# NagsTheProgrammer/WindGNN

Measured on NVIDIA B200. Metric: gcn_gru_forward_sequences_per_s, higher is better.
Workload: dtype f32

## Files before the change

windgnn_b200/csrc/abi.cu:

```cuda

#include "../../include/windgnn_b200.h"

#include <cmath>
#include <cstdarg>
#include <cstdio>
#include <cstdlib>
#include <cstring>
#include <mutex>
#include <vector>

#include "gcn.cuh"
#include "gcn_bwd.cuh"
#include "gcn_bwd_rows.cuh"
#include "gcn_rows.cuh"
#include "gcn_sparse.cuh"
#include "gcn_sparse_plan.cuh"
#include "gemm_kb.cuh"
#include "gru_bwd.cuh"
#include "inproj.cuh"
#include "inproj_tc2.cuh"
#include "recur.cuh"
#include "recur_tc.cuh"
#include "recur_unit.cuh"
#include "sgemm.cuh"
// ... 35 lines not shown

constexpr size_t kAlign = 256;
size_t align_up(size_t v) { return (v + kAlign - 1) / kAlign * kAlign; }

enum GcnKind { kGcnRows, kGcn13x7, kGcn13x4, kGcn16x4, kGcnSparsePlan, kGcnSparseLanes };
enum RecurKind { kRecurTc, kRecurUnit, kRecurWide };

struct Plan {
    int T, S, Fi, Fh, Fo, H;
    long long chunk;
    int I, G;
    int IP;
    int NPB;
    int GP;
    int KP;
    int NPR;
    int n_bias;
    bool sparse;
    GcnKind gcn;
    size_t gcn_smem;
    int gcn_rb;
    int gcn_threads;
    size_t off_sqw, off_sqsteps, off_sqpairs;
    bool tc;
    wg::Tc2Shape tc2;
    RecurKind recur;
    bool regw;
    bool whu;
    int ru_wpg, ru_ht;
    int ru_rmax;
    int rc_ts;
    size_t rc_smem;
    size_t off_wp, off_bias, off_wht, off_whu, off_bhn, off_u, off_gi, off_z, total;
    size_t off_whh_hi, off_whh_lo;
};

long long default_chunk(long long B, size_t bytes_per_seq) {
    long long c = (long long)wg::kNumSMs * wg::kRcBT;
    const size_t cap = (size_t)6 << 30;
    if ((size_t)c * bytes_per_seq > cap) {
        c = (long long)(cap / bytes_per_seq) / wg::kRcBT * wg::kRcBT;
        if (c < wg::kRcBT) c = wg::kRcBT;
    }
    return B < c ? (B < 1 ? 1 : B) : c;
}

// ... 92 lines not shown
    const int wrows = p.tc && p.tc2.NP > p.NPB ? p.tc2.NP : p.NPB;
    p.n_bias = wrows > 512 ? wrows : 512;
    p.off_wp = o;   o = align_up(o + (p.tc ? wg::tc2_w_halves(p.tc2) * 2 : (size_t)p.NPB * p.IP * 4));
    p.off_bias = o; o = align_up(o + (size_t)p.n_bias * 4);
    p.off_wht = o;  o = align_up(o + (size_t)p.KP * p.NPR * 4);
    p.off_whu = o;
    if (p.whu) o = align_up(o + (size_t)p.KP * 3 * wg::recur_u_hp2(H) * 4);
    p.off_bhn = o;  o = align_up(o + (size_t)p.KP * 4);
    const bool tc_recur = p.recur == kRecurTc;
    p.off_whh_hi = o; if (tc_recur) o = align_up(o + wg::recur_tc_w_halves(H) * 2);
    p.off_whh_lo = o; if (tc_recur) o = align_up(o + wg::recur_tc_w_halves(H) * 2);
    const size_t rows = table_rows > 0 ? (size_t)forecast_piece_rows(p, table_rows) : (size_t)p.chunk * T;
    const size_t rows_tiled = (rows + wg::kUTileRows - 1) / wg::kUTileRows * wg::kUTileRows;
    p.off_u = o;    o = align_up(o + rows_tiled * p.IP * 4);
    const size_t rows_gi =
        table_rows > 0 ? (size_t)table_rows : (size_t)((p.chunk + wg::kRtSeqs - 1) / wg::kRtSeqs * wg::kRtSeqs) * T;
    p.off_gi = o;   o = align_up(o + rows_gi * p.GP * 4);
    p.off_z = o;    if (sparse) o = align_up(o + (rows + wg::kNumSMs) * (size_t)S * Fo * 4);
    const bool sq = p.gcn == kGcnSparsePlan;
    p.off_sqw = o;     if (sq) o = align_up(o + sizeof(wg::SqWeights));
    p.off_sqsteps = o;
    p.off_sqpairs = o + (size_t)wg::round_up(wg::ceil_div(S, 32), 4) * sizeof(int);
    if (sq) o = align_up(o + wg::sq_plan_bytes(S));
    p.total = o;
    return WG_OK;
}

int plan_launch(Plan& p) {
    const long long rows = p.chunk * p.T;
    switch (p.gcn) {
    case kGcnRows:
        p.gcn_smem = wg::gcn_rows_smem_floats(p.S) * 4;
        p.gcn_threads = wg::gcn_rows_warps(p.S) * 32;
        break;
    case kGcnSparsePlan: {
        p.gcn_smem = wg::gcn_sparse_plan_smem_bytes(p.S, p.Fi, p.Fo);
        const long long rt = (rows + wg::kSpThreads - 1) / wg::kSpThreads * wg::kSpThreads;
        if (rt / 32 > 65535) return fail(WG_ERR_UNSUPPORTED, "sparse GCN: chunk of %lld rows too large", rows);
        break;
    }
    case kGcnSparseLanes:
        if (p.Fi > wg::kSpF || p.Fo > wg::kSpF)
            return fail(WG_ERR_UNSUPPORTED, "sparse GCN: F_in / F_out must be <= %d (got %d / %d)", wg::kSpF, p.Fi, p.Fo);
        p.gcn_smem = ((size_t)2 * p.Fh * wg::kSpF + p.Fh) * 4;
        if (p.gcn_smem > (size_t)wg::kMaxSmemOptin)
            return fail(WG_ERR_UNSUPPORTED, "sparse GCN: hidden width %d too large", p.Fh);
// ... 88 lines not shown
    WG_CUDA(cudaOccupancyMaxActiveBlocksPerMultiprocessor(&per_sm, kern, wg::kGcnThreads, smem));
    if (per_sm < 1) per_sm = 1;
    const long long nblocks = (R + RB - 1) / RB;
    long long grid = (long long)wg::kNumSMs * per_sm;
    if (grid > nblocks) grid = nblocks;
    if (grid < 1) return WG_OK;
    kern<<<(unsigned)grid, wg::kGcnThreads, smem, st>>>(X, adj, W1, b1, W2, b2, out, R, S, Fi, Fh, Fo, ldo, RB);
    WG_CUDA(cudaGetLastError());
    return WG_OK;
}

template <int LAYERS, bool TILED>
int launch_gcn_dense(GcnKind k, int RB, size_t smem, const float* X, const float* adj, const float* W1,
                     const float* b1, const float* W2, const float* b2, float* out, long long R, int S, int Fi, int Fh,
                     int Fo, int ldo, cudaStream_t st) {
#define WG_GCN(FP, SG, EX) \
    launch_gcn_t<FP, SG, EX, LAYERS, TILED>(X, adj, W1, b1, W2, b2, out, R, S, Fi, Fh, Fo, ldo, RB, smem, st)
    if (k == kGcn13x7) return WG_GCN(13, 7, true);
    if (k == kGcn13x4) return WG_GCN(13, 4, true);
    return WG_GCN(16, 4, false);
#undef WG_GCN
}

int launch_gcn_rows(const Plan& p, const float* X, const float* adj, const float* W1, const float* b1,
                    const float* W2, const float* b2, float* out, long long R, cudaStream_t st) {
    WG_CUDA(cudaFuncSetAttribute(wg::gcn_rows_kernel, cudaFuncAttributeMaxDynamicSharedMemorySize, (int)p.gcn_smem));
    int per_sm = 0;
    WG_CUDA(cudaOccupancyMaxActiveBlocksPerMultiprocessor(&per_sm, wg::gcn_rows_kernel, p.gcn_threads, p.gcn_smem));
    if (per_sm < 1) per_sm = 1;
    const long long nblocks = (R + wg::kGrRows - 1) / wg::kGrRows;
    long long grid = (long long)wg::kNumSMs * per_sm;
    if (grid > nblocks) grid = nblocks;
    if (grid < 1) return WG_OK;
    wg::gcn_rows_kernel<<<(unsigned)grid, p.gcn_threads, p.gcn_smem, st>>>(X, adj, W1, b1, W2, b2, out, R, p.S, p.IP);
    WG_CUDA(cudaGetLastError());
    return WG_OK;
}

struct Graph {
    const float* adj;
    const int* rowptr;
    const int* colidx;
    const float* vals;
};

int launch_gcn_sparse(const Plan& p, void* ws, const Graph& g, const float* x, const float* w1, const float* b1,
                      const float* w2, const float* b2, long long rows, cudaStream_t st) {
    if (rows < 1) return WG_OK;
    if (p.gcn == kGcnSparsePlan) {
        const bool narrow = p.Fi <= 13 && p.Fo <= 13, exact = p.Fi == 13 && p.Fo == 13;
        auto kern = exact ? wg::gcn_sparse_plan_kernel<13, true>
                          : narrow ? wg::gcn_sparse_plan_kernel<13, false> : wg::gcn_sparse_plan_kernel<16, false>;
        WG_CUDA(cudaFuncSetAttribute(kern, cudaFuncAttributeMaxDynamicSharedMemorySize, (int)p.gcn_smem));
        const unsigned grid = (unsigned)(rows < wg::kNumSMs ? rows : wg::kNumSMs);
        float* urow = ws_ptr<float>(ws, p.off_z);
        float* zscr = urow + (size_t)rows * p.S * p.Fo;
        kern<<<grid, wg::kSqThreads, p.gcn_smem, st>>>(x, g.rowptr, g.colidx, g.vals, ws_ptr<int>(ws, p.off_sqsteps),
// ... 10 lines not shown
    }
    const long long tiles = (rows + wg::kSpThreads - 1) / wg::kSpThreads;
    int chunks = (int)((4LL * wg::kNumSMs * 4 + tiles - 1) / tiles);
    if (chunks < 1) chunks = 1;
    if (chunks > p.S) chunks = p.S;
    const int s_chunk = (p.S + chunks - 1) / chunks;
    const dim3 grid((unsigned)tiles, (unsigned)((p.S + s_chunk - 1) / s_chunk));
    WG_CUDA(cudaFuncSetAttribute(wg::gcn_sparse_l1_kernel, cudaFuncAttributeMaxDynamicSharedMemorySize,
                                 (int)p.gcn_smem));
    wg::gcn_sparse_l1_kernel<<<grid, wg::kSpThreads, p.gcn_smem, st>>>(x, g.rowptr, g.colidx, g.vals, w1, b1, w2,
                                                                       ws_ptr<float>(ws, p.off_z), rows, p.S, p.Fi,
                                                                       p.Fh, p.Fo, s_chunk);
    WG_CUDA(cudaGetLastError());
    wg::gcn_sparse_l2_kernel<<<grid, wg::kSpThreads, 0, st>>>(ws_ptr<float>(ws, p.off_z), g.rowptr, g.colidx, g.vals,
                                                             b2, ws_ptr<float>(ws, p.off_u), rows, p.S, p.Fo, p.IP,
                                                             s_chunk);
    WG_CUDA(cudaGetLastError());
    return WG_OK;
}

int launch_gcn(const Plan& p, void* ws, const Graph& g, const float* x, const float* w1, const float* b1,
               const float* w2, const float* b2, long long rows, cudaStream_t st) {
    float* u = ws_ptr<float>(ws, p.off_u);
    if (p.gcn == kGcnRows) return launch_gcn_rows(p, x, g.adj, w1, b1, w2, b2, u, rows, st);
    if (p.sparse) return launch_gcn_sparse(p, ws, g, x, w1, b1, w2, b2, rows, st);
    return launch_gcn_dense<2, true>(p.gcn, p.gcn_rb, p.gcn_smem, x, g.adj, w1, b1, w2, b2, u, rows, p.S, p.Fi, p.Fh,
                                     p.Fo, p.IP, st);
}

int launch_inproj_tc(const Plan& p, void* ws, long long rows, cudaStream_t st, float* gi) {
    const long long m_tiles = (rows + wg::kT2BM - 1) / wg::kT2BM;
    if (m_tiles < 1) return WG_OK;
    const wg::Tc2Shape& t = p.tc2;
    WG_CUDA(cudaFuncSetAttribute(wg::inproj_tc2_kernel, cudaFuncAttributeMaxDynamicSharedMemorySize,
                                 (int)t.smem_bytes));
    const long long tiles = m_tiles * t.n_nt;
    const unsigned grid = (unsigned)(tiles < wg::kNumSMs ? tiles : wg::kNumSMs);
    wg::inproj_tc2_kernel<<<grid, wg::kT2Threads, t.smem_bytes, st>>>(
        ws_ptr<float>(ws, p.off_u), ws_ptr<__half>(ws, p.off_wp), ws_ptr<float>(ws, p.off_bias), gi, rows, p.IP,
        t.KP, p.GP, t.n_nt, t.N_each, t.stages);
    WG_CUDA(cudaGetLastError());
    return WG_OK;
}

int launch_inproj(const Plan& p, void* ws, long long rows, cudaStream_t st, float* gi) {
    if (p.tc) return launch_inproj_tc(p, ws, rows, st, gi);
    const long long m_tiles = (rows + wg::kIpBM - 1) / wg::kIpBM;
// ... 135 lines not shown
                                                           ws_ptr<__half>(ws, p.off_whh_lo), p.H);
        WG_CUDA(cudaGetLastError());
    }
    return WG_OK;
}

int run_chunk(const Plan& p, void* ws, const Graph& g, const float* x, const float* w1, const float* b1,
              const float* w2, const float* b2, float* out, long long Bc, cudaStream_t st, float* gsave = nullptr,
              int ldsave = 0) {
    const long long rows = Bc * p.T;
    int rc = launch_gcn(p, ws, g, x, w1, b1, w2, b2, rows, st);
    if (rc) return rc;
    rc = launch_inproj(p, ws, rows, st, ws_ptr<float>(ws, p.off_gi));
    if (rc) return rc;
    return launch_recur(p, ws, out, Bc, st, gsave, ldsave);
}

constexpr int kMaxDevices = 64;

std::mutex g_sq_mu;
struct SqDeviceState { cudaEvent_t ev = nullptr; cudaStream_t last = nullptr; bool recorded = false; };
SqDeviceState g_sq_dev[kMaxDevices];

int prepare_sparse(const Plan& p, void* ws, const Graph& g, const float* w1, const float* b1, const float* w2,
                   const float* b2, int device, cudaStream_t st) {
    if (device >= kMaxDevices) return fail(WG_ERR_BAD_ARG, "device index %d out of range", device);
    wg::SqWeights* stage = ws_ptr<wg::SqWeights>(ws, p.off_sqw);
    wg::sq_pack_weights_kernel<<<32, 256, 0, st>>>(w1, b1, w2, b2, stage, p.Fi, p.Fh, p.Fo);
    WG_CUDA(cudaGetLastError());
    const int wbs = wg::ceil_div(p.S, 32);
    wg::csr_plan_kernel<<<wg::ceil_div(wbs, 4), 128, 0, st>>>(g.rowptr, g.colidx, g.vals, p.S,
                                                             ws_ptr<int>(ws, p.off_sqsteps),
                                                             ws_ptr<int2>(ws, p.off_sqpairs));
    WG_CUDA(cudaGetLastError());
    SqDeviceState& d = g_sq_dev[device];
    cudaStreamCaptureStatus cap = cudaStreamCaptureStatusNone;
    cudaStreamIsCapturing(st, &cap);
    if (cap == cudaStreamCaptureStatusNone && d.recorded && d.last != st) WG_CUDA(cudaStreamWaitEvent(st, d.ev, 0));
    WG_CUDA(cudaMemcpyToSymbolAsync(wg::c_sq, stage, sizeof(wg::SqWeights), 0, cudaMemcpyDeviceToDevice, st));
    return WG_OK;
}
int finish_sparse(int device, cudaStream_t st) {
    SqDeviceState& d = g_sq_dev[device];
    cudaStreamCaptureStatus cap = cudaStreamCaptureStatusNone;
    cudaStreamIsCapturing(st, &cap);
    if (cap != cudaStreamCaptureStatusNone) return WG_OK;
    if (!d.ev) WG_CUDA(cudaEventCreateWithFlags(&d.ev, cudaEventDisableTiming));
    WG_CUDA(cudaEventRecord(d.ev, st));
    d.last = st;
    d.recorded = true;
    return WG_OK;
}

bool any_null(std::initializer_list<const void*> ps) {
    for (const void* q : ps)
        if (!q) return true;
    return false;
}

template <typename Stages>
int run_packed(const Plan& p, size_t need, const Graph& g, const float* x, const float* w1, const float* b1,
               const float* w2, const float* b2, const float* w_ih, const float* w_hh, const float* b_ih,
               const float* b_hh, const float* out, void* ws, size_t ws_bytes, int device, void* stream,
               Stages stages) {
    const bool no_graph = p.sparse ? any_null({g.rowptr, g.colidx, g.vals}) : !g.adj;
    if (no_graph || any_null({x, w1, b1, w2, b2, w_ih, w_hh, b_ih, b_hh, out}))
        return fail(WG_ERR_BAD_ARG, "null pointer argument");
    int rc = check_ws(ws, ws_bytes, need);
    if (rc) return rc;
    DeviceGuard dg(device);
    WG_CUDA(dg.err);
    cudaStream_t st = static_cast<cudaStream_t>(stream);
    if ((rc = launch_pack(p, ws, w_ih, w_hh, b_ih, b_hh, st))) return rc;
    const bool sq = p.gcn == kGcnSparsePlan;
    std::unique_lock<std::mutex> sq_lock(g_sq_mu, std::defer_lock);
    if (sq) {
        sq_lock.lock();
        if ((rc = prepare_sparse(p, ws, g, w1, b1, w2, b2, device, st))) return rc;
    }
    if ((rc = stages(st))) return rc;
    return sq ? finish_sparse(device, st) : WG_OK;
}

int forward(const Plan& p, size_t need, const Graph& g, const float* x, const float* w1, const float* b1,
            const float* w2, const float* b2, const float* w_ih, const float* w_hh, const float* b_ih,
            const float* b_hh, float* out, long long B, void* ws, size_t ws_bytes, int device, void* stream,
            float* gsave = nullptr, int ldsave = 0) {
    if (B == 0) return WG_OK;
    auto stages = [&](cudaStream_t st) {
        const size_t x_seq = (size_t)p.T * p.S * p.Fi, o_seq = (size_t)p.T * p.H;
        for (long long b0 = 0; b0 < B; b0 += p.chunk) {
            const long long Bc = (B - b0) < p.chunk ? (B - b0) : p.chunk;
            const int rc = run_chunk(p, ws, g, x + (size_t)b0 * x_seq, w1, b1, w2, b2, out + (size_t)b0 * o_seq, Bc,
                                     st, gsave ? gsave + (size_t)b0 * p.T * ldsave : nullptr, ldsave);
            if (rc) return rc;
        }
        return (int)WG_OK;
    };
    return run_packed(p, need, g, x, w1, b1, w2, b2, w_ih, w_hh, b_ih, b_hh, out, ws, ws_bytes, device, stream,
                      stages);
}

struct ForecastPlan {
    Plan p;
// ... 265 lines not shown
int wg_internal_fail(int code, const char* msg) { return fail(code, "%s", msg); }
const char* wg_last_error(void) { return g_err; }

size_t wg_gcn_gru_workspace_bytes(int64_t B, int T, int S, int F_in, int F_hid, int F_out, int H,
                                  int64_t chunk, int flags) {
    Plan p;
    if (make_plan(p, B, T, S, F_in, F_hid, F_out, H, chunk, false, flags)) return 0;
    return p.total;
}

int wg_stage_pack_f32(const float* w_ih, const float* w_hh, const float* b_ih, const float* b_hh, int T,
                      int S, int F_in, int F_hid, int F_out, int H, int64_t chunk, int flags, void* workspace,
                      size_t workspace_bytes, int device, void* stream) {
    if (any_null({w_ih, w_hh, b_ih, b_hh})) return fail(WG_ERR_BAD_ARG, "null parameter pointer");
    auto launch = [&](const Plan& p, cudaStream_t st) { return launch_pack(p, workspace, w_ih, w_hh, b_ih, b_hh, st); };
    return run_stage(0, T, S, F_in, F_hid, F_out, H, chunk, flags, workspace, workspace_bytes, device, stream, launch);
}

int wg_stage_gcn_f32(const float* adj, const float* x, const float* w1, const float* b1, const float* w2,
                     const float* b2, int64_t Bc, int T, int S, int F_in, int F_hid, int F_out, int H,
                     int64_t chunk, int flags, void* workspace, size_t workspace_bytes, int device, void* stream) {
    if (any_null({adj, x, w1, b1, w2, b2})) return fail(WG_ERR_BAD_ARG, "null pointer");
    auto launch = [&](const Plan& p, cudaStream_t st) {
        return launch_gcn(p, workspace, Graph{adj}, x, w1, b1, w2, b2, Bc * T, st);
    };
    return run_stage(Bc, T, S, F_in, F_hid, F_out, H, chunk, flags, workspace, workspace_bytes, device, stream, launch);
}

int wg_stage_inproj_f32(int64_t Bc, int T, int S, int F_in, int F_hid, int F_out, int H, int64_t chunk,
                        int flags, void* workspace, size_t workspace_bytes, int device, void* stream) {
    auto launch = [&](const Plan& p, cudaStream_t st) {
        return launch_inproj(p, workspace, Bc * T, st, ws_ptr<float>(workspace, p.off_gi));
    };
    return run_stage(Bc, T, S, F_in, F_hid, F_out, H, chunk, flags, workspace, workspace_bytes, device, stream, launch);
}

int wg_stage_recur_f32(float* out, int64_t Bc, int T, int S, int F_in, int F_hid, int F_out, int H,
                       int64_t chunk, int flags, void* workspace, size_t workspace_bytes, int device, void* stream) {
    if (!out) return fail(WG_ERR_BAD_ARG, "null output pointer");
    auto launch = [&](const Plan& p, cudaStream_t st) { return launch_recur(p, workspace, out, Bc, st, nullptr, 0); };
    return run_stage(Bc, T, S, F_in, F_hid, F_out, H, chunk, flags, workspace, workspace_bytes, device, stream, launch);
}

int wg_gcn_gru_forward_f32(const float* adj, const float* x, const float* w1, const float* b1,
                           const float* w2, const float* b2, const float* w_ih, const float* w_hh,
                           const float* b_ih, const float* b_hh, float* out, int64_t B, int T, int S,
                           int F_in, int F_hid, int F_out, int H, int64_t chunk, int flags, void* workspace,
// ... 137 lines not shown
    float* pdev[kHostSlots];
    for (int i = 0; i < kHostSlots; ++i) {
        xdev[i] = reinterpret_cast<float*>(slots + i * L.xs);
        odev[i] = reinterpret_cast<float*>(slots + kHostSlots * L.xs + i * L.os);
        pdev[i] = reinterpret_cast<float*>(slots + kHostSlots * (L.xs + L.os) + i * L.ps);
    }
    int result = WG_OK;
#define WG_CUDA_H(expr)                                                                         \
    do {                                                                                        \
        cudaError_t e_ = (expr);                                                                \
        if (e_ != cudaSuccess) {                                                                \
            result = fail(WG_ERR_CUDA, "%s failed: %s (%s:%d)", #expr, cudaGetErrorString(e_),  \
                          __FILE__, __LINE__);                                                  \
            cudaDeviceSynchronize();                                                            \
            return result;                                                                      \
        }                                                                                       \
    } while (0)

    auto synced = [](int code) { cudaDeviceSynchronize(); return code; };
    const long long n_chunks = (B + p.chunk - 1) / p.chunk;
    for (int l = 0; l < kHostLanes && l < n_chunks; ++l)
        if ((rc = launch_pack(p, lane_ws[l], w_ih, w_hh, b_ih, b_hh, cx->s_cmp[l]))) return synced(rc);
    const Graph graph{adj};
    const size_t x_seq = (size_t)T * S * F_in, o_seq = (size_t)T * H;
    for (long long c = 0; c < n_chunks; ++c) {
        const int sl = (int)(c % kHostSlots), lane = (int)(c % kHostLanes);
        const long long b0 = c * p.chunk;
        const long long Bc = (B - b0) < p.chunk ? (B - b0) : p.chunk;
        if (c >= kHostSlots) WG_CUDA_H(cudaStreamWaitEvent(cx->s_in, cx->ev_cmp[sl], 0));
        WG_CUDA_H(cudaMemcpyAsync(xdev[sl], x_host + (size_t)b0 * x_seq, (size_t)Bc * x_seq * 4,
                                  cudaMemcpyHostToDevice, cx->s_in));
        WG_CUDA_H(cudaEventRecord(cx->ev_in[sl], cx->s_in));
        WG_CUDA_H(cudaStreamWaitEvent(cx->s_cmp[lane], cx->ev_in[sl], 0));
        if (c >= kHostSlots) WG_CUDA_H(cudaStreamWaitEvent(cx->s_cmp[lane], cx->ev_out[sl], 0));
        if ((rc = run_chunk(p, lane_ws[lane], graph, xdev[sl], w1, b1, w2, b2, odev[sl], Bc, cx->s_cmp[lane])))
            return synced(rc);
        if (last_only &&
            (rc = wg_denorm_last_step_f32(odev[sl], pdev[sl], Bc, T, H, vmin, vmax, device, cx->s_cmp[lane])))
            return synced(rc);
        WG_CUDA_H(cudaEventRecord(cx->ev_cmp[sl], cx->s_cmp[lane]));
        WG_CUDA_H(cudaStreamWaitEvent(cx->s_out, cx->ev_cmp[sl], 0));
        if (last_only)
            WG_CUDA_H(cudaMemcpyAsync(dst_host + (size_t)b0 * H, pdev[sl], (size_t)Bc * H * 4, cudaMemcpyDeviceToHost,
                                      cx->s_out));
        else
            WG_CUDA_H(cudaMemcpyAsync(dst_host + (size_t)b0 * o_seq, odev[sl], (size_t)Bc * o_seq * 4,
// ... 274 lines not shown
```

windgnn_b200/csrc/gcn_rows.cuh:

```cuda
#pragma once

#include "gcn.cuh"
#include "wg_common.cuh"

namespace wg {

constexpr int kGrRows = 32;
constexpr int kGrF = 13;
constexpr int kGrFS = 16;
constexpr int kGrAP = 12;
constexpr int kGrMaxPairs = 5;
constexpr int kGrMaxWarps = 8;

__host__ __device__ inline int gcn_rows_warps(int S) { return ceil_div(ceil_div(S, 2), kGrMaxPairs); }
__host__ __device__ inline bool gcn_rows_applies(int S, int Fi, int Fh, int Fo) {
    return Fi == kGrF && Fh == kGrF && Fo == kGrF && gcn_rows_warps(S) <= kGrMaxWarps && S <= 48;
}
__host__ __device__ inline int gcn_rows_rs2(int S) { return S * kGrFS + 4; }
constexpr int kGrXS = 28;
__host__ __device__ inline bool gcn_rows_balanced(int S) { return ceil_div(S, 2) == 17; }
constexpr int kGrSliceStep = 3;
constexpr int kGrSliceW = 4;
__host__ __device__ inline size_t gcn_rows_smem_floats(int S) {
    const int NW = gcn_rows_warps(S);
    size_t n = (size_t)S * NW * kGrAP;
    n += 2 * (size_t)kGcnFS * kGcnFS + 2 * kGcnFS;
    const size_t in_f = (size_t)kGrRows * S * kGrF, g1_f = (size_t)kGrRows * gcn_rows_rs2(S);
    n += round_up((int)(in_f > g1_f ? in_f : g1_f), 4) + 4;
    if (gcn_rows_balanced(S)) n += 2 * (size_t)kGrRows * kGrXS;
    return n;
}

template <int NPW, bool SHARED>
struct GrFrag {
    static constexpr int NA4 = (NPW + (SHARED ? 1 : 0) + 1) / 2;
    float a[NA4 * 4];
    float x[kGrF];
    float xs[kGrSliceW];
};

template <int NPW, bool PADDED, bool VEC, bool SHARED>
__device__ __forceinline__ void gr_aggregate_x(float2 (&acc)[NPW][kGrF], float2 (&accs)[4],
                                               const float* __restrict__ xrow, const float* __restrict__ arow,
                                               int astride, int S, int fs0) {
    using Frag = GrFrag<NPW, SHARED>;
#pragma unroll
    for (int j = 0; j < 4; ++j) accs[j] = make_float2(0.0f, 0.0f);
#pragma unroll
    for (int p = 0; p < NPW; ++p)
#pragma unroll
        for (int f = 0; f < kGrF; ++f) acc[p][f] = make_float2(0.0f, 0.0f);
    auto load = [&](Frag& fr, int sp, auto odd_tag) {
        constexpr bool ODD = decltype(odd_tag)::value != 0;
        const float* ap = arow + (size_t)sp * astride;
#pragma unroll
        for (int q = 0; q < Frag::NA4; ++q) {
            const float4 t = *reinterpret_cast<const float4*>(ap + 4 * q);
            fr.a[4 * q] = t.x; fr.a[4 * q + 1] = t.y; fr.a[4 * q + 2] = t.z; fr.a[4 * q + 3] = t.w;
        }
        if constexpr (SHARED) {
            const float* xq = xrow + sp * (PADDED ? kGrFS : kGrF) + fs0;
#pragma unroll
            for (int j = 0; j < kGrSliceW; ++j) fr.xs[j] = xq[j];
        }
        if (PADDED) {
            const float* xp = xrow + sp * kGrFS;
#pragma unroll
            for (int q = 0; q < 3; ++q) {
                const float4 t = *reinterpret_cast<const float4*>(xp + 4 * q);
                fr.x[4 * q] = t.x; fr.x[4 * q + 1] = t.y; fr.x[4 * q + 2] = t.z; fr.x[4 * q + 3] = t.w;
            }
            fr.x[12] = xp[12];
        } else {
            const float* xp = xrow + sp * kGrF;
            if (!VEC) {
#pragma unroll
                for (int f = 0; f < kGrF; ++f) fr.x[f] = xp[f];
            } else if (!ODD) {
#pragma unroll
                for (int q = 0; q < 6; ++q) {
                    const float2 t = *reinterpret_cast<const float2*>(xp + 2 * q);
                    fr.x[2 * q] = t.x; fr.x[2 * q + 1] = t.y;
                }
                fr.x[12] = xp[12];
            } else {
                fr.x[0] = xp[0];
#pragma unroll
                for (int q = 0; q < 6; ++q) {
                    const float2 t = *reinterpret_cast<const float2*>(xp + 1 + 2 * q);
                    fr.x[1 + 2 * q] = t.x; fr.x[2 + 2 * q] = t.y;
                }
            }
        }
    };
    auto fma = [&](const Frag& fr) {
#pragma unroll
        for (int p = 0; p < NPW; ++p) {
            const float2 aa = make_float2(fr.a[2 * p], fr.a[2 * p + 1]);
#pragma unroll
            for (int f = 0; f < kGrF; ++f) acc[p][f] = __ffma2_rn(make_float2(fr.x[f], fr.x[f]), aa, acc[p][f]);
        }
        if constexpr (SHARED) {
            const float2 aa = make_float2(fr.a[2 * NPW], fr.a[2 * NPW + 1]);
#pragma unroll
            for (int j = 0; j < kGrSliceW; ++j) accs[j] = __ffma2_rn(make_float2(fr.xs[j], fr.xs[j]), aa, accs[j]);
        }
    };
    Frag f0, f1;
    load(f0, 0, IntC<0>{});
    int sp = 0;
#pragma unroll 1
    for (; sp + 2 < S; sp += 2) {
        load(f1, sp + 1, IntC<1>{});
        fma(f0);
        load(f0, sp + 2, IntC<0>{});
        fma(f1);
    }
    if (sp + 1 < S) {
        load(f1, sp + 1, IntC<1>{});
        fma(f0);
        fma(f1);
    } else {
        fma(f0);
    }
}

template <int NPW, bool PADDED, bool VEC>
__device__ __forceinline__ void gr_aggregate(float2 (&acc)[NPW][kGrF], const float* __restrict__ xrow,
                                             const float* __restrict__ arow, int astride, int S) {
    float2 unused[4];
    gr_aggregate_x<NPW, PADDED, VEC, false>(acc, unused, xrow, arow, astride, S, 0);
}

__device__ __forceinline__ void gr_transform_shared(float2 (&o)[kGrSliceW], const float* __restrict__ xrow,
                                                    const float* __restrict__ Wn, int c0) {
    float2 agg[kGrF + 1];
#pragma unroll
    for (int q = 0; q < 7; ++q) {
        const float4 t = *reinterpret_cast<const float4*>(xrow + 4 * q);
        agg[2 * q] = make_float2(t.x, t.y);
        agg[2 * q + 1] = make_float2(t.z, t.w);
    }
#pragma unroll
    for (int j = 0; j < kGrSliceW; ++j) o[j] = make_float2(0.0f, 0.0f);
    const float* wp = Wn + c0;
#pragma unroll
// ... 28 lines not shown
    asm("max.NaN.f32 %0, %1, 0f00000000;" : "=f"(r) : "f"(u));
    return r;
}
__device__ __forceinline__ float2 gr_bias(float2 o, float b) { return __fadd2_rn(o, make_float2(b, b)); }

template <int NPW, bool SHARED>
__device__ __forceinline__ void gr_block(float* __restrict__ buf, const float* __restrict__ arow, int astride,
                                         const float* __restrict__ w1d, const float* __restrict__ b1s,
                                         const float* __restrict__ w2d, const float* __restrict__ b2s, int S, int s0,
                                         int lane, bool row_ok, float* __restrict__ out_col0, int ldo, bool pad_warp,
                                         const float* __restrict__ next_src, unsigned next_bytes, uint64_t* bar,
                                         float* __restrict__ xch, int f0) {
    constexpr int SNF = kGrSliceW;
    constexpr int SS = 32;
    const int SF0 = f0;
    const int in_cols = S * kGrF, RS2 = gcn_rows_rs2(S);
    float2 acc[NPW][kGrF];
    float2 accs[4];
    auto put_shared = [&](float* row) {
#pragma unroll
        for (int j = 0; j < SNF; ++j) *reinterpret_cast<float2*>(row + 2 * (SF0 + j)) = accs[j];
    };
    if ((in_cols & 1) == 0)
        gr_aggregate_x<NPW, false, true, SHARED>(acc, accs, buf + (size_t)lane * in_cols, arow, astride, S, f0);
    else
        gr_aggregate_x<NPW, false, false, SHARED>(acc, accs, buf + (size_t)lane * in_cols, arow, astride, S, f0);
    if (SHARED) put_shared(xch);
    __syncthreads();
    float* g1row = buf + (size_t)lane * RS2;
    auto store_g1 = [&](const float2 (&o)[NPW][4], int c0) {
        const float4 bb = *reinterpret_cast<const float4*>(b1s + c0);
        const float bv[4] = {bb.x, bb.y, bb.z, bb.w};
#pragma unroll
        for (int p = 0; p < NPW; ++p) {
            const int s = s0 + 2 * p;
            float4 v0, v1;
            const float2 u0 = gr_bias(o[p][0], bv[0]), u1 = gr_bias(o[p][1], bv[1]);
            const float2 u2 = gr_bias(o[p][2], bv[2]), u3 = gr_bias(o[p][3], bv[3]);
            v0.x = gr_relu(u0.x); v0.y = gr_relu(u1.x); v0.z = gr_relu(u2.x); v0.w = gr_relu(u3.x);
            v1.x = gr_relu(u0.y); v1.y = gr_relu(u1.y); v1.z = gr_relu(u2.y); v1.w = gr_relu(u3.y);
            *reinterpret_cast<float4*>(g1row + s * kGrFS + c0) = v0;
            if (s + 1 < S) *reinterpret_cast<float4*>(g1row + (s + 1) * kGrFS + c0) = v1;
        }
    };
    {
        float2 o[NPW][4];
#pragma unroll 1
        for (int c0 = 0; c0 < 12; c0 += 4) {
            gr_transform_chunk<NPW, 4>(o, acc, w1d, c0);
            store_g1(o, c0);
        }
        gr_transform_chunk<NPW, 1>(o, acc, w1d, 12);
        store_g1(o, 12);
    }
    if (SHARED) {
        float2 o[4];
        gr_transform_shared(o, xch, w1d, SF0);
#pragma unroll
        for (int j = 0; j < SNF; ++j) {
            const float2 u = gr_bias(o[j], b1s[SF0 + j]);
            g1row[SS * kGrFS + SF0 + j] = gr_relu(u.x);
            if (SS + 1 < S) g1row[(SS + 1) * kGrFS + SF0 + j] = gr_relu(u.y);
        }
    }
    __syncthreads();
    gr_aggregate_x<NPW, true, true, SHARED>(acc, accs, g1row, arow, astride, S, f0);
    if (SHARED) put_shared(xch + kGrRows * kGrXS);
    __syncthreads();
    if (next_bytes != 0 && threadIdx.x == 0) {
        mbar_expect_tx(bar, next_bytes);
        bulk_g2s(buf, next_src, next_bytes, bar);
    }
    auto store_u = [&](const float2 (&o)[NPW][4], int c0, auto width) {
        constexpr int W = decltype(width)::value;
        const float4 bb = *reinterpret_cast<const float4*>(b2s + c0);
        const float bv[4] = {bb.x, bb.y, bb.z, bb.w};
        if (row_ok) {
#pragma unroll
            for (int p = 0; p < NPW; ++p) {
                const int s = s0 + 2 * p;
                float* c_lo = out_col0 + (size_t)(s * kGrF + c0) * kUTileRows;
#pragma unroll
                for (int c = 0; c < W; ++c) {
                    const float2 u = gr_bias(o[p][c], bv[c]);
                    c_lo[(size_t)c * kUTileRows] = gr_relu(u.x);
                    if (s + 1 < S) c_lo[(size_t)(kGrF + c) * kUTileRows] = gr_relu(u.y);
                }
            }
        }
    };
    {
        float2 o[NPW][4];
#pragma unroll 1
        for (int c0 = 0; c0 < 12; c0 += 4) {
            gr_transform_chunk<NPW, 4>(o, acc, w2d, c0);
            store_u(o, c0, IntC<4>{});
        }
        gr_transform_chunk<NPW, 1>(o, acc, w2d, 12);
        store_u(o, 12, IntC<1>{});
    }
    if (SHARED) {
        float2 o[4];
        gr_transform_shared(o, xch + kGrRows * kGrXS, w2d, SF0);
        if (row_ok) {
            float* c_lo = out_col0 + (size_t)(SS * kGrF + SF0) * kUTileRows;
#pragma unroll
            for (int j = 0; j < SNF; ++j) {
                const float2 u = gr_bias(o[j], b2s[SF0 + j]);
                c_lo[(size_t)j * kUTileRows] = gr_relu(u.x);
                if (SS + 1 < S) c_lo[(size_t)(kGrF + j) * kUTileRows] = gr_relu(u.y);
            }
        }
    }
    if (pad_warp && row_ok)
        for (int c = in_cols; c < ldo; ++c) out_col0[(size_t)c * kUTileRows] = 0.0f;
}

__global__ void __launch_bounds__(kGrMaxWarps * 32, 1)
    gcn_rows_kernel(const float* __restrict__ X, const float* __restrict__ adj, const float* __restrict__ W1,
                    const float* __restrict__ b1, const float* __restrict__ W2, const float* __restrict__ b2,
                    float* __restrict__ out, long long R, int S, int ldo) {
    extern __shared__ __align__(16) float smem[];
    const int NW = gcn_rows_warps(S);
    const int nthreads = NW * 32;
    const int tid = threadIdx.x, lane = tid & 31;
    const int in_cols = S * kGrF;
    const bool balanced = gcn_rows_balanced(S);
    const int NPT = balanced ? 16 : ceil_div(S, 2), base = NPT / NW, extra = NPT % NW;
    const int w = ((tid >> 5) + (blockIdx.x / kNumSMs) * 2) % NW;
    const int npw = base + (w < extra ? 1 : 0);
    const int p0 = w * base + (w < extra ? w : extra);
    const int s0 = 2 * p0;

    float* adjW = smem;
    float* w1d = adjW + (size_t)S * NW * kGrAP;
    float* w2d = w1d + kGcnFS * kGcnFS;
    float* b1s = w2d + kGcnFS * kGcnFS;
    float* b2s = b1s + kGcnFS;
    float* buf = b2s + kGcnFS;
    const size_t in_f = (size_t)kGrRows * in_cols, g1_f = (size_t)kGrRows * gcn_rows_rs2(S);
    uint64_t* bar = reinterpret_cast<uint64_t*>(buf + round_up((int)(in_f > g1_f ? in_f : g1_f), 4));
    float* xch = reinterpret_cast<float*>(bar) + 4 + (size_t)lane * kGrXS;

    for (int e = tid; e < S * NW * kGrAP; e += nthreads) {
        const int sp = e / (NW * kGrAP), c = e % (NW * kGrAP);
        const int ww = c / kGrAP, i = c % kGrAP;
        const int wn = base + (ww < extra ? 1 : 0), ws0 = 2 * (ww * base + (ww < extra ? ww : extra));
        const int s = i < 2 * wn ? ws0 + i : (balanced && i < 2 * wn + 2 ? 32 + (i - 2 * wn) : S);
        adjW[e] = s < S ? adj[(size_t)s * S + sp] : 0.0f;
    }
    for (int e = tid; e < kGcnFS * kGcnFS; e += nthreads) {
        const int f = e / kGcnFS, fo = e % kGcnFS;
        const bool in = f < kGrF && fo < kGrF;
        w1d[e] = in ? W1[f * kGrF + fo] : 0.0f;
        w2d[e] = in ? W2[f * kGrF + fo] : 0.0f;
    }
    for (int e = tid; e < kGcnFS; e += nthreads) {
        b1s[e] = e < kGrF ? b1[e] : 0.0f;
        b2s[e] = e < kGrF ? b2[e] : 0.0f;
    }
    if (tid == 0) {
        mbar_init(bar, 1);
        fence_mbar_init();
    }
    __syncthreads();

    const float* arow = adjW + w * kGrAP;
    const int astride = NW * kGrAP;
    const long long nblocks = (R + kGrRows - 1) / kGrRows;
    unsigned phase = 0;
    auto block_span = [&](long long rb, const float*& src, unsigned& bytes, int& nrows) {
        const long long r0 = rb * kGrRows;
        nrows = (int)((R - r0) < kGrRows ? (R - r0) : kGrRows);
        src = X + (size_t)r0 * in_cols;
        bytes = (unsigned)((size_t)nrows * in_cols * 4);
        return ((reinterpret_cast<uintptr_t>(src) & 15) == 0) && ((bytes & 15) == 0);
    };
    bool prefetched = false;
    for (long long rb = blockIdx.x; rb < nblocks; rb += gridDim.x) {
        const long long r0 = rb * kGrRows;
        const float* src;
        unsigned bytes;
        int nrows;
        const bool bulk = block_span(rb, src, bytes, nrows);
        if (bulk) {
            if (!prefetched && tid == 0) {
                mbar_expect_tx(bar, bytes);
                bulk_g2s(buf, src, bytes, bar);
            }
            mbar_wait(bar, phase);
// ... 36 lines not shown
```

Before: 776,900.

## Move GCN-rows adjacency and weights into constant memory via a pack kernel

The dense rows GCN kernel now reads its adjacency slices, weights and biases from a __constant__ struct filled by a separate pack kernel and a device-to-device symbol copy, instead of staging them into shared memory in every block. Because the warp index is made uniform with a reduce, adjacency reads become uniform constant-cache broadcasts. The shared layer-1 row stride is narrowed from 16 to 14 floats, with float2 accesses replacing float4, and the kernel's register cap changes from launch bounds to __maxnreg__. This cuts shared-memory footprint and per-block setup, but adds a serialized pack-and-copy step under a global mutex, and every entry path has to call prepare/finish.

```diff
diff --git a/windgnn_b200/csrc/abi.cu b/windgnn_b200/csrc/abi.cu
--- a/windgnn_b200/csrc/abi.cu
+++ b/windgnn_b200/csrc/abi.cu
@@ -81,6 +81,7 @@
     int gcn_rb;
     int gcn_threads;
     size_t off_sqw, off_sqsteps, off_sqpairs;
+    size_t off_grw;
     bool tc;
     wg::Tc2Shape tc2;
     RecurKind recur;
@@ -219,6 +220,7 @@
     p.off_sqsteps = o;
     p.off_sqpairs = o + (size_t)wg::round_up(wg::ceil_div(S, 32), 4) * sizeof(int);
     if (sq) o = align_up(o + wg::sq_plan_bytes(S));
+    p.off_grw = o;     if (p.gcn == kGcnRows) o = align_up(o + sizeof(wg::GrParams));
     p.total = o;
     return WG_OK;
 }
@@ -353,8 +355,7 @@
 #undef WG_GCN
 }
 
-int launch_gcn_rows(const Plan& p, const float* X, const float* adj, const float* W1, const float* b1,
-                    const float* W2, const float* b2, float* out, long long R, cudaStream_t st) {
+int launch_gcn_rows(const Plan& p, const float* X, float* out, long long R, cudaStream_t st) {
     WG_CUDA(cudaFuncSetAttribute(wg::gcn_rows_kernel, cudaFuncAttributeMaxDynamicSharedMemorySize, (int)p.gcn_smem));
     int per_sm = 0;
     WG_CUDA(cudaOccupancyMaxActiveBlocksPerMultiprocessor(&per_sm, wg::gcn_rows_kernel, p.gcn_threads, p.gcn_smem));
@@ -363,7 +364,7 @@
     long long grid = (long long)wg::kNumSMs * per_sm;
     if (grid > nblocks) grid = nblocks;
     if (grid < 1) return WG_OK;
-    wg::gcn_rows_kernel<<<(unsigned)grid, p.gcn_threads, p.gcn_smem, st>>>(X, adj, W1, b1, W2, b2, out, R, p.S, p.IP);
+    wg::gcn_rows_kernel<<<(unsigned)grid, p.gcn_threads, p.gcn_smem, st>>>(X, out, R, p.S, p.IP);
     WG_CUDA(cudaGetLastError());
     return WG_OK;
 }
@@ -420,7 +421,7 @@
 int launch_gcn(const Plan& p, void* ws, const Graph& g, const float* x, const float* w1, const float* b1,
                const float* w2, const float* b2, long long rows, cudaStream_t st) {
     float* u = ws_ptr<float>(ws, p.off_u);
-    if (p.gcn == kGcnRows) return launch_gcn_rows(p, x, g.adj, w1, b1, w2, b2, u, rows, st);
+    if (p.gcn == kGcnRows) return launch_gcn_rows(p, x, u, rows, st);
     if (p.sparse) return launch_gcn_sparse(p, ws, g, x, w1, b1, w2, b2, rows, st);
     return launch_gcn_dense<2, true>(p.gcn, p.gcn_rb, p.gcn_smem, x, g.adj, w1, b1, w2, b2, u, rows, p.S, p.Fi, p.Fh,
                                      p.Fo, p.IP, st);
@@ -602,25 +603,42 @@
 struct SqDeviceState { cudaEvent_t ev = nullptr; cudaStream_t last = nullptr; bool recorded = false; };
 SqDeviceState g_sq_dev[kMaxDevices];
 
-int prepare_sparse(const Plan& p, void* ws, const Graph& g, const float* w1, const float* b1, const float* w2,
-                   const float* b2, int device, cudaStream_t st) {
+bool uses_const(const Plan& p) { return p.gcn == kGcnSparsePlan || p.gcn == kGcnRows; }
+
+int prepare_const(const Plan& p, void* ws, const Graph& g, const float* w1, const float* b1, const float* w2,
+                  const float* b2, int device, cudaStream_t st) {
     if (device >= kMaxDevices) return fail(WG_ERR_BAD_ARG, "device index %d out of range", device);
-    wg::SqWeights* stage = ws_ptr<wg::SqWeights>(ws, p.off_sqw);
-    wg::sq_pack_weights_kernel<<<32, 256, 0, st>>>(w1, b1, w2, b2, stage, p.Fi, p.Fh, p.Fo);
-    WG_CUDA(cudaGetLastError());
-    const int wbs = wg::ceil_div(p.S, 32);
-    wg::csr_plan_kernel<<<wg::ceil_div(wbs, 4), 128, 0, st>>>(g.rowptr, g.colidx, g.vals, p.S,
-                                                             ws_ptr<int>(ws, p.off_sqsteps),
-                                                             ws_ptr<int2>(ws, p.off_sqpairs));
-    WG_CUDA(cudaGetLastError());
+    const void* stage;
+    size_t bytes;
+    if (p.gcn == kGcnRows) {
+        wg::GrParams* gs = ws_ptr<wg::GrParams>(ws, p.off_grw);
+        wg::gr_pack_kernel<<<8, 256, 0, st>>>(g.adj, w1, b1, w2, b2, gs, p.S);
+        WG_CUDA(cudaGetLastError());
+        stage = gs;
+        bytes = sizeof(wg::GrParams);
+    } else {
+        wg::SqWeights* sq = ws_ptr<wg::SqWeights>(ws, p.off_sqw);
+        wg::sq_pack_weights_kernel<<<32, 256, 0, st>>>(w1, b1, w2, b2, sq, p.Fi, p.Fh, p.Fo);
+        WG_CUDA(cudaGetLastError());
+        const int wbs = wg::ceil_div(p.S, 32);
+        wg::csr_plan_kernel<<<wg::ceil_div(wbs, 4), 128, 0, st>>>(g.rowptr, g.colidx, g.vals, p.S,
+                                                                 ws_ptr<int>(ws, p.off_sqsteps),
+                                                                 ws_ptr<int2>(ws, p.off_sqpairs));
+        WG_CUDA(cudaGetLastError());
+        stage = sq;
+        bytes = sizeof(wg::SqWeights);
+    }
     SqDeviceState& d = g_sq_dev[device];
     cudaStreamCaptureStatus cap = cudaStreamCaptureStatusNone;
     cudaStreamIsCapturing(st, &cap);
     if (cap == cudaStreamCaptureStatusNone && d.recorded && d.last != st) WG_CUDA(cudaStreamWaitEvent(st, d.ev, 0));
-    WG_CUDA(cudaMemcpyToSymbolAsync(wg::c_sq, stage, sizeof(wg::SqWeights), 0, cudaMemcpyDeviceToDevice, st));
-    return WG_OK;
-}
-int finish_sparse(int device, cudaStream_t st) {
+    if (p.gcn == kGcnRows)
+        WG_CUDA(cudaMemcpyToSymbolAsync(wg::c_gr, stage, bytes, 0, cudaMemcpyDeviceToDevice, st));
+    else
+        WG_CUDA(cudaMemcpyToSymbolAsync(wg::c_sq, stage, bytes, 0, cudaMemcpyDeviceToDevice, st));
+    return WG_OK;
+}
+int finish_const(int device, cudaStream_t st) {
     SqDeviceState& d = g_sq_dev[device];
     cudaStreamCaptureStatus cap = cudaStreamCaptureStatusNone;
     cudaStreamIsCapturing(st, &cap);
@@ -652,14 +670,14 @@
     WG_CUDA(dg.err);
     cudaStream_t st = static_cast<cudaStream_t>(stream);
     if ((rc = launch_pack(p, ws, w_ih, w_hh, b_ih, b_hh, st))) return rc;
-    const bool sq = p.gcn == kGcnSparsePlan;
-    std::unique_lock<std::mutex> sq_lock(g_sq_mu, std::defer_lock);
-    if (sq) {
-        sq_lock.lock();
-        if ((rc = prepare_sparse(p, ws, g, w1, b1, w2, b2, device, st))) return rc;
+    const bool cb = uses_const(p);
+    std::unique_lock<std::mutex> cb_lock(g_sq_mu, std::defer_lock);
+    if (cb) {
+        cb_lock.lock();
+        if ((rc = prepare_const(p, ws, g, w1, b1, w2, b2, device, st))) return rc;
     }
     if ((rc = stages(st))) return rc;
-    return sq ? finish_sparse(device, st) : WG_OK;
+    return cb ? finish_const(device, st) : WG_OK;
 }
 
 int forward(const Plan& p, size_t need, const Graph& g, const float* x, const float* w1, const float* b1,
@@ -971,7 +989,15 @@
                      int64_t chunk, int flags, void* workspace, size_t workspace_bytes, int device, void* stream) {
     if (any_null({adj, x, w1, b1, w2, b2})) return fail(WG_ERR_BAD_ARG, "null pointer");
     auto launch = [&](const Plan& p, cudaStream_t st) {
-        return launch_gcn(p, workspace, Graph{adj}, x, w1, b1, w2, b2, Bc * T, st);
+        const Graph g{adj};
+        std::unique_lock<std::mutex> cb_lock(g_sq_mu, std::defer_lock);
+        int rc;
+        if (uses_const(p)) {
+            cb_lock.lock();
+            if ((rc = prepare_const(p, workspace, g, w1, b1, w2, b2, device, st))) return rc;
+        }
+        if ((rc = launch_gcn(p, workspace, g, x, w1, b1, w2, b2, Bc * T, st))) return rc;
+        return uses_const(p) ? finish_const(device, st) : WG_OK;
     };
     return run_stage(Bc, T, S, F_in, F_hid, F_out, H, chunk, flags, workspace, workspace_bytes, device, stream, launch);
 }
@@ -1155,6 +1181,13 @@
     for (int l = 0; l < kHostLanes && l < n_chunks; ++l)
         if ((rc = launch_pack(p, lane_ws[l], w_ih, w_hh, b_ih, b_hh, cx->s_cmp[l]))) return synced(rc);
     const Graph graph{adj};
+    std::unique_lock<std::mutex> cb_lock(g_sq_mu, std::defer_lock);
+    if (uses_const(p)) {
+        cb_lock.lock();
+        if ((rc = prepare_const(p, lane_ws[0], graph, w1, b1, w2, b2, device, cx->s_cmp[0]))) return synced(rc);
+        if ((rc = finish_const(device, cx->s_cmp[0]))) return synced(rc);
+        for (int l = 1; l < kHostLanes; ++l) WG_CUDA_H(cudaStreamWaitEvent(cx->s_cmp[l], g_sq_dev[device].ev, 0));
+    }
     const size_t x_seq = (size_t)T * S * F_in, o_seq = (size_t)T * H;
     for (long long c = 0; c < n_chunks; ++c) {
         const int sl = (int)(c % kHostSlots), lane = (int)(c % kHostLanes);
diff --git a/windgnn_b200/csrc/gcn_rows.cuh b/windgnn_b200/csrc/gcn_rows.cuh
--- a/windgnn_b200/csrc/gcn_rows.cuh
+++ b/windgnn_b200/csrc/gcn_rows.cuh
@@ -7,28 +7,72 @@
 
 constexpr int kGrRows = 32;
 constexpr int kGrF = 13;
-constexpr int kGrFS = 16;
+constexpr int kGrFS = 14;
 constexpr int kGrAP = 12;
 constexpr int kGrMaxPairs = 5;
 constexpr int kGrMaxWarps = 8;
+constexpr int kGrMaxS = 48;
+constexpr int kGrMaxRegs = 168;
 
 __host__ __device__ inline int gcn_rows_warps(int S) { return ceil_div(ceil_div(S, 2), kGrMaxPairs); }
 __host__ __device__ inline bool gcn_rows_applies(int S, int Fi, int Fh, int Fo) {
-    return Fi == kGrF && Fh == kGrF && Fo == kGrF && gcn_rows_warps(S) <= kGrMaxWarps && S <= 48;
-}
-__host__ __device__ inline int gcn_rows_rs2(int S) { return S * kGrFS + 4; }
+    return Fi == kGrF && Fh == kGrF && Fo == kGrF && gcn_rows_warps(S) <= kGrMaxWarps && S <= kGrMaxS;
+}
+__host__ __device__ inline int gcn_rows_rs2(int S) { return S * kGrFS + ((S * kGrFS) % 4 == 0 ? 2 : 0); }
 constexpr int kGrXS = 28;
 __host__ __device__ inline bool gcn_rows_balanced(int S) { return ceil_div(S, 2) == 17; }
 constexpr int kGrSliceStep = 3;
 constexpr int kGrSliceW = 4;
 __host__ __device__ inline size_t gcn_rows_smem_floats(int S) {
-    const int NW = gcn_rows_warps(S);
-    size_t n = (size_t)S * NW * kGrAP;
-    n += 2 * (size_t)kGcnFS * kGcnFS + 2 * kGcnFS;
+    size_t n = 0;
     const size_t in_f = (size_t)kGrRows * S * kGrF, g1_f = (size_t)kGrRows * gcn_rows_rs2(S);
     n += round_up((int)(in_f > g1_f ? in_f : g1_f), 4) + 4;
     if (gcn_rows_balanced(S)) n += 2 * (size_t)kGrRows * kGrXS;
     return n;
+}
+
+struct __align__(16) GrParams {
+    float adj[kGrMaxS * kGrMaxWarps * kGrAP];
+    float w1[kGcnFS * kGcnFS];
+    float w2[kGcnFS * kGcnFS];
+    float b1[kGcnFS];
+    float b2[kGcnFS];
+};
+__constant__ GrParams c_gr;
+
+__host__ __device__ inline void gcn_rows_pairs(int S, int w, int& npw, int& p0) {
+    const int NW = gcn_rows_warps(S);
+    const int NPT = gcn_rows_balanced(S) ? 16 : ceil_div(S, 2), base = NPT / NW, extra = NPT % NW;
+    npw = base + (w < extra ? 1 : 0);
+    p0 = w * base + (w < extra ? w : extra);
+}
+
+__global__ void gr_pack_kernel(const float* __restrict__ adj, const float* __restrict__ W1,
+                               const float* __restrict__ b1, const float* __restrict__ W2,
+                               const float* __restrict__ b2, GrParams* __restrict__ dst, int S) {
+    const int NW = gcn_rows_warps(S);
+    const bool balanced = gcn_rows_balanced(S);
+    const int stride = gridDim.x * blockDim.x;
+    const int t0 = blockIdx.x * blockDim.x + threadIdx.x;
+    for (int e = t0; e < S * NW * kGrAP; e += stride) {
+        const int sp = e / (NW * kGrAP), c = e % (NW * kGrAP);
+        const int ww = c / kGrAP, i = c % kGrAP;
+        int wn, wp0;
+        gcn_rows_pairs(S, ww, wn, wp0);
+        const int ws0 = 2 * wp0;
+        const int s = i < 2 * wn ? ws0 + i : (balanced && i < 2 * wn + 2 ? 32 + (i - 2 * wn) : S);
+        dst->adj[e] = s < S ? adj[(size_t)s * S + sp] : 0.0f;
+    }
+    for (int e = t0; e < kGcnFS * kGcnFS; e += stride) {
+        const int f = e / kGcnFS, fo = e % kGcnFS;
+        const bool in = f < kGrF && fo < kGrF;
+        dst->w1[e] = in ? W1[f * kGrF + fo] : 0.0f;
+        dst->w2[e] = in ? W2[f * kGrF + fo] : 0.0f;
+    }
+    for (int e = t0; e < kGcnFS; e += stride) {
+        dst->b1[e] = e < kGrF ? b1[e] : 0.0f;
+        dst->b2[e] = e < kGrF ? b2[e] : 0.0f;
+    }
 }
 
 template <int NPW, bool SHARED>
@@ -39,7 +83,7 @@
     float xs[kGrSliceW];
 };
 
-template <int NPW, bool PADDED, bool VEC, bool SHARED>
+template <int NPW, bool PADDED, bool VEC, bool SHARED, bool CONSTA = false>
 __device__ __forceinline__ void gr_aggregate_x(float2 (&acc)[NPW][kGrF], float2 (&accs)[4],
                                                const float* __restrict__ xrow, const float* __restrict__ arow,
                                                int astride, int S, int fs0) {
@@ -52,11 +96,13 @@
         for (int f = 0; f < kGrF; ++f) acc[p][f] = make_float2(0.0f, 0.0f);
     auto load = [&](Frag& fr, int sp, auto odd_tag) {
         constexpr bool ODD = decltype(odd_tag)::value != 0;
-        const float* ap = arow + (size_t)sp * astride;
-#pragma unroll
-        for (int q = 0; q < Frag::NA4; ++q) {
-            const float4 t = *reinterpret_cast<const float4*>(ap + 4 * q);
-            fr.a[4 * q] = t.x; fr.a[4 * q + 1] = t.y; fr.a[4 * q + 2] = t.z; fr.a[4 * q + 3] = t.w;
+        if constexpr (!CONSTA) {
+            const float* ap = arow + (size_t)sp * astride;
+#pragma unroll
+            for (int q = 0; q < Frag::NA4; ++q) {
+                const float4 t = *reinterpret_cast<const float4*>(ap + 4 * q);
+                fr.a[4 * q] = t.x; fr.a[4 * q + 1] = t.y; fr.a[4 * q + 2] = t.z; fr.a[4 * q + 3] = t.w;
+            }
         }
         if constexpr (SHARED) {
             const float* xq = xrow + sp * (PADDED ? kGrFS : kGrF) + fs0;
@@ -66,9 +112,9 @@
         if (PADDED) {
             const float* xp = xrow + sp * kGrFS;
 #pragma unroll
-            for (int q = 0; q < 3; ++q) {
-                const float4 t = *reinterpret_cast<const float4*>(xp + 4 * q);
-                fr.x[4 * q] = t.x; fr.x[4 * q + 1] = t.y; fr.x[4 * q + 2] = t.z; fr.x[4 * q + 3] = t.w;
+            for (int q = 0; q < 6; ++q) {
+                const float2 t = *reinterpret_cast<const float2*>(xp + 2 * q);
+                fr.x[2 * q] = t.x; fr.x[2 * q + 1] = t.y;
             }
             fr.x[12] = xp[12];
         } else {
@@ -93,15 +139,23 @@
             }
         }
     };
-    auto fma = [&](const Frag& fr) {
+    auto adj_pair = [&](const Frag& fr, int sp, int i) {
+        if constexpr (CONSTA) {
+            const float* ap = arow + sp * astride;
+            return make_float2(ap[i], ap[i + 1]);
+        } else {
+            return make_float2(fr.a[i], fr.a[i + 1]);
+        }
+    };
+    auto fma = [&](const Frag& fr, int sp) {
 #pragma unroll
         for (int p = 0; p < NPW; ++p) {
-            const float2 aa = make_float2(fr.a[2 * p], fr.a[2 * p + 1]);
+            const float2 aa = adj_pair(fr, sp, 2 * p);
 #pragma unroll
             for (int f = 0; f < kGrF; ++f) acc[p][f] = __ffma2_rn(make_float2(fr.x[f], fr.x[f]), aa, acc[p][f]);
         }
         if constexpr (SHARED) {
-            const float2 aa = make_float2(fr.a[2 * NPW], fr.a[2 * NPW + 1]);
+            const float2 aa = adj_pair(fr, sp, 2 * NPW);
 #pragma unroll
             for (int j = 0; j < kGrSliceW; ++j) accs[j] = __ffma2_rn(make_float2(fr.xs[j], fr.xs[j]), aa, accs[j]);
         }
@@ -112,16 +166,16 @@
 #pragma unroll 1
     for (; sp + 2 < S; sp += 2) {
         load(f1, sp + 1, IntC<1>{});
-        fma(f0);
+        fma(f0, sp);
         load(f0, sp + 2, IntC<0>{});
-        fma(f1);
+        fma(f1, sp + 1);
     }
     if (sp + 1 < S) {
         load(f1, sp + 1, IntC<1>{});
-        fma(f0);
-        fma(f1);
+        fma(f0, sp);
+        fma(f1, sp + 1);
     } else {
-        fma(f0);
+        fma(f0, sp);
     }
 }
 
@@ -196,25 +250,35 @@
         for (int j = 0; j < SNF; ++j) *reinterpret_cast<float2*>(row + 2 * (SF0 + j)) = accs[j];
     };
     if ((in_cols & 1) == 0)
-        gr_aggregate_x<NPW, false, true, SHARED>(acc, accs, buf + (size_t)lane * in_cols, arow, astride, S, f0);
+        gr_aggregate_x<NPW, false, true, SHARED, true>(acc, accs, buf + (size_t)lane * in_cols, arow, astride, S, f0);
     else
-        gr_aggregate_x<NPW, false, false, SHARED>(acc, accs, buf + (size_t)lane * in_cols, arow, astride, S, f0);
+        gr_aggregate_x<NPW, false, false, SHARED, true>(acc, accs, buf + (size_t)lane * in_cols, arow, astride, S, f0);
     if (SHARED) put_shared(xch);
     __syncthreads();
     float* g1row = buf + (size_t)lane * RS2;
-    auto store_g1 = [&](const float2 (&o)[NPW][4], int c0) {
-        const float4 bb = *reinterpret_cast<const float4*>(b1s + c0);
-        const float bv[4] = {bb.x, bb.y, bb.z, bb.w};
+    auto store_g1 = [&](const float2 (&o)[NPW][4], int c0, auto width) {
+        constexpr int W = decltype(width)::value;
+        constexpr int NV = W == 4 ? 4 : 2;
+        float bv[NV];
+#pragma unroll
+        for (int c = 0; c < NV; ++c) bv[c] = b1s[c0 + c];
 #pragma unroll
         for (int p = 0; p < NPW; ++p) {
             const int s = s0 + 2 * p;
-            float4 v0, v1;
-            const float2 u0 = gr_bias(o[p][0], bv[0]), u1 = gr_bias(o[p][1], bv[1]);
-            const float2 u2 = gr_bias(o[p][2], bv[2]), u3 = gr_bias(o[p][3], bv[3]);
-            v0.x = gr_relu(u0.x); v0.y = gr_relu(u1.x); v0.z = gr_relu(u2.x); v0.w = gr_relu(u3.x);
-            v1.x = gr_relu(u0.y); v1.y = gr_relu(u1.y); v1.z = gr_relu(u2.y); v1.w = gr_relu(u3.y);
-            *reinterpret_cast<float4*>(g1row + s * kGrFS + c0) = v0;
-            if (s + 1 < S) *reinterpret_cast<float4*>(g1row + (s + 1) * kGrFS + c0) = v1;
+            float v0[NV], v1[NV];
+#pragma unroll
+            for (int c = 0; c < NV; ++c) {
+                const float2 u = gr_bias(o[p][c], bv[c]);
+                v0[c] = gr_relu(u.x);
+                v1[c] = gr_relu(u.y);
+            }
+#pragma unroll
+            for (int q = 0; q < NV / 2; ++q) {
+                *reinterpret_cast<float2*>(g1row + s * kGrFS + c0 + 2 * q) = make_float2(v0[2 * q], v0[2 * q + 1]);
+                if (s + 1 < S)
+                    *reinterpret_cast<float2*>(g1row + (s + 1) * kGrFS + c0 + 2 * q) =
+                        make_float2(v1[2 * q], v1[2 * q + 1]);
+            }
         }
     };
     {
@@ -222,10 +286,10 @@
 #pragma unroll 1
         for (int c0 = 0; c0 < 12; c0 += 4) {
             gr_transform_chunk<NPW, 4>(o, acc, w1d, c0);
-            store_g1(o, c0);
+            store_g1(o, c0, IntC<4>{});
         }
         gr_transform_chunk<NPW, 1>(o, acc, w1d, 12);
-        store_g1(o, 12);
+        store_g1(o, 12, IntC<1>{});
     }
     if (SHARED) {
         float2 o[4];
@@ -238,7 +302,7 @@
         }
     }
     __syncthreads();
-    gr_aggregate_x<NPW, true, true, SHARED>(acc, accs, g1row, arow, astride, S, f0);
+    gr_aggregate_x<NPW, true, true, SHARED, true>(acc, accs, g1row, arow, astride, S, f0);
     if (SHARED) put_shared(xch + kGrRows * kGrXS);
     __syncthreads();
     if (next_bytes != 0 && threadIdx.x == 0) {
@@ -247,8 +311,9 @@
     }
     auto store_u = [&](const float2 (&o)[NPW][4], int c0, auto width) {
         constexpr int W = decltype(width)::value;
-        const float4 bb = *reinterpret_cast<const float4*>(b2s + c0);
-        const float bv[4] = {bb.x, bb.y, bb.z, bb.w};
+        float bv[W];
+#pragma unroll
+        for (int c = 0; c < W; ++c) bv[c] = b2s[c0 + c];
         if (row_ok) {
 #pragma unroll
             for (int p = 0; p < NPW; ++p) {
@@ -290,56 +355,32 @@
         for (int c = in_cols; c < ldo; ++c) out_col0[(size_t)c * kUTileRows] = 0.0f;
 }
 
-__global__ void __launch_bounds__(kGrMaxWarps * 32, 1)
-    gcn_rows_kernel(const float* __restrict__ X, const float* __restrict__ adj, const float* __restrict__ W1,
-                    const float* __restrict__ b1, const float* __restrict__ W2, const float* __restrict__ b2,
-                    float* __restrict__ out, long long R, int S, int ldo) {
+__global__ void __maxnreg__(kGrMaxRegs)
+    gcn_rows_kernel(const float* __restrict__ X, float* __restrict__ out, long long R, int S, int ldo) {
     extern __shared__ __align__(16) float smem[];
     const int NW = gcn_rows_warps(S);
     const int nthreads = NW * 32;
     const int tid = threadIdx.x, lane = tid & 31;
     const int in_cols = S * kGrF;
     const bool balanced = gcn_rows_balanced(S);
-    const int NPT = balanced ? 16 : ceil_div(S, 2), base = NPT / NW, extra = NPT % NW;
-    const int w = ((tid >> 5) + (blockIdx.x / kNumSMs) * 2) % NW;
-    const int npw = base + (w < extra ? 1 : 0);
-    const int p0 = w * base + (w < extra ? w : extra);
+    const int w = (int)__reduce_min_sync(0xffffffffu, (unsigned)(((tid >> 5) + (blockIdx.x / kNumSMs) * 2) % NW));
+    int npw, p0;
+    gcn_rows_pairs(S, w, npw, p0);
     const int s0 = 2 * p0;
 
-    float* adjW = smem;
-    float* w1d = adjW + (size_t)S * NW * kGrAP;
-    float* w2d = w1d + kGcnFS * kGcnFS;
-    float* b1s = w2d + kGcnFS * kGcnFS;
-    float* b2s = b1s + kGcnFS;
-    float* buf = b2s + kGcnFS;
+    float* buf = smem;
     const size_t in_f = (size_t)kGrRows * in_cols, g1_f = (size_t)kGrRows * gcn_rows_rs2(S);
     uint64_t* bar = reinterpret_cast<uint64_t*>(buf + round_up((int)(in_f > g1_f ? in_f : g1_f), 4));
     float* xch = reinterpret_cast<float*>(bar) + 4 + (size_t)lane * kGrXS;
 
-    for (int e = tid; e < S * NW * kGrAP; e += nthreads) {
-        const int sp = e / (NW * kGrAP), c = e % (NW * kGrAP);
-        const int ww = c / kGrAP, i = c % kGrAP;
-        const int wn = base + (ww < extra ? 1 : 0), ws0 = 2 * (ww * base + (ww < extra ? ww : extra));
-        const int s = i < 2 * wn ? ws0 + i : (balanced && i < 2 * wn + 2 ? 32 + (i - 2 * wn) : S);
-        adjW[e] = s < S ? adj[(size_t)s * S + sp] : 0.0f;
-    }
-    for (int e = tid; e < kGcnFS * kGcnFS; e += nthreads) {
-        const int f = e / kGcnFS, fo = e % kGcnFS;
-        const bool in = f < kGrF && fo < kGrF;
-        w1d[e] = in ? W1[f * kGrF + fo] : 0.0f;
-        w2d[e] = in ? W2[f * kGrF + fo] : 0.0f;
-    }
-    for (int e = tid; e < kGcnFS; e += nthreads) {
-        b1s[e] = e < kGrF ? b1[e] : 0.0f;
-        b2s[e] = e < kGrF ? b2[e] : 0.0f;
-    }
     if (tid == 0) {
         mbar_init(bar, 1);
         fence_mbar_init();
     }
     __syncthreads();
 
-    const float* arow = adjW + w * kGrAP;
+    const float* arow = c_gr.adj + w * kGrAP;
+    const float *w1d = c_gr.w1, *w2d = c_gr.w2, *b1s = c_gr.b1, *b2s = c_gr.b2;
     const int astride = NW * kGrAP;
     const long long nblocks = (R + kGrRows - 1) / kGrRows;
     unsigned phase = 0;
```

Result: faster. 791,900, median of 6 (+1.9%).
